# ffahleraz/rllib-warehouse

Hardware: AMD Instinct MI355X
Metric: agent-steps/sec (aggregate) at B=65536 envs × 8 agents, 1/2/4/8 MI355X (higher is better)
Workload: dtype u8/u32 packed integer state, f32 rewards

## Files before the change

### rllib-warehouse_amd/csrc/device_vocab.h

```cpp
constexpr int BT = 256;
using PkCell = uint16_t;
constexpr uint32_t PKW = sizeof(PkCell);
constexpr uint32_t ROWB = PKW * BT;

enum Policy { POL_EXTERNAL = 0, POL_GREEDY = 1, POL_RANDOM = 2 };
enum Purpose : uint32_t { PUR_RESET = 1, PUR_REGEN = 2, PUR_POLICY = 3, PUR_RANDOM = 4 };
constexpr int PH_ALL = 0, PH_PRE = 1, PH_REGEN = 2, PH_POLICY = 3;
#ifdef WH_ABLATION
constexpr bool kAblationBuild = true;
#else
constexpr bool kAblationBuild = false;
#endif

#ifndef WH_OBS_EB0
#define WH_OBS_EB0 4
#endif
constexpr int kObsEB[4] = {WH_OBS_EB0, 8, 16, 64};
#ifndef WH_OBS_CHUNK
#define WH_OBS_CHUNK 1024
#endif
constexpr int kObsChunk = WH_OBS_CHUNK;
#ifndef WH_FUSE_ROWS_MAX
#define WH_FUSE_ROWS_MAX 4096
#endif
// ... 148 lines not shown
}

__device__ __forceinline__ uint32_t action_of(uint32_t d) {
  const short2v v = as_s2(d);
  return (uint32_t)(3 * ((int)v.x + 1) + ((int)v.y + 1));
}

#define WH_RARE(x) __builtin_expect(!!(x), 0)

#ifdef WH_PHASE_MARKS
#define WH_PHASE_MARK(name) asm volatile("; PHASE " #name ::: "memory")
#else
#define WH_PHASE_MARK(name) ((void)0)
#endif

template <class C>
struct Regs {
  uint32_t hdr, epi;
  uint32_t ag[C::NAM];
  uint64_t am;
  uint32_t wskip;
};

template <class C>
struct Lds {
  alignas(16) uint32_t tbl[4 * C::TBL4];
  uint32_t occ[C::D][BT];
  PkCell pkp[C::P + 1][BT];
  alignas(16) uint32_t agl[C::NAM][BT];
  __device__ __forceinline__ uint32_t cell_row(uint32_t xy16) const {
    if constexpr (cell_skew(C::D)) {
      const uint32_t i = __builtin_amdgcn_udot4(xy16, 0x00840004u, 0u, false);
      return reinterpret_cast<const uint8_t*>(tbl)[i];
    } else {
      return reinterpret_cast<const uint8_t*>(tbl)[__builtin_amdgcn_perm(xy16, xy16, 0x0C0C0200u)];
    }
  }

  __device__ __forceinline__ uint2 rtag(uint32_t j) const {
    return reinterpret_cast<const uint2*>(&tbl[C::T.rp / 4])[j];
  }
  __device__ __forceinline__ uint32_t mv(uint32_t a) const { return tbl[C::T.mv / 4 + a]; }
  __device__ __forceinline__ uint32_t valid_cell(uint32_t v) const { return tbl[C::T.valid / 4 + v]; }
  __device__ __forceinline__ uint32_t target_byte(uint32_t j, int tid) const {
    return *reinterpret_cast<const uint8_t*>(&pkp[j][tid]);
  }
  __device__ __forceinline__ void clear_target(uint32_t j, int tid) {
    *reinterpret_cast<uint8_t*>(&pkp[j][tid]) = 0;
  }
  __device__ __forceinline__ uint32_t pkp_offset() const {
    return (uint32_t)(reinterpret_cast<const char*>(&pkp[0][0]) - reinterpret_cast<const char*>(this));
  }
  __device__ __forceinline__ const uint8_t* row_byte(uint32_t cv, int tid) const {
    return reinterpret_cast<const uint8_t*>(this) + (pkp_offset() - ROWB) + cv * ROWB + PKW * tid;
  }
  __device__ __forceinline__ uint8_t* row_byte(uint32_t cv, int tid) {
    return reinterpret_cast<uint8_t*>(this) + (pkp_offset() - ROWB) + cv * ROWB + PKW * tid;
  }
  __device__ __forceinline__ uint32_t dst_tb(uint32_t tb) const { return tbl[C::T.dst / 4 - 1 + tb]; }
};

template <class C>
struct Slots {
  uint32_t rs_ag[C::NAM][BT];
  uint16_t rs_req[C::R][BT];
  uint32_t rs_am[2][BT], rs_hdr[BT], rs_ep[BT];
};
struct NoSlots {};

template <class C>
constexpr int kTableChunks = (C::TBL4 + BT - 1) / BT;
template <class C>
__device__ __forceinline__ bool table_lane(int i) {
// ... 76 lines not shown
  for (int w = 0; w < C::PW; ++w) {
    const uint32_t lo = __builtin_amdgcn_perm(r.pm[w], r.pt[w], 0x05010400u);
    const uint32_t hi = __builtin_amdgcn_perm(r.pm[w], r.pt[w], 0x07030602u);
    L.pkp[4 * w][tid] = (uint16_t)lo;
    L.pkp[4 * w + 1][tid] = (uint16_t)(lo >> 16);
    L.pkp[4 * w + 2][tid] = (uint16_t)hi;
    L.pkp[4 * w + 3][tid] = (uint16_t)(hi >> 16);
  }
  s.am = active_mask<C>(r.pt);
  const uint32_t t0 = s.hdr & 0xFFFFu;
  const uint32_t thr = t0 < W ? W - t0 : 0u;
  uint32_t early = 0;
#pragma unroll
  for (int w = 0; w < C::PW; ++w)
    early |= nz_hi(r.pt[w]) & swar_lt(swar_sub(r.pm[w], (t0 & 0xFFu) * 0x01010101u), thr * 0x01010101u);
  s.wskip = __any(early != 0u) ? 0u : W;
}

template <class C>
__device__ __forceinline__ void store_env(const Regs<C>& s, const Lds<C>& L, uint32_t* __restrict__ st,
                                          int64_t B, int64_t e0, int na, int tid) {
  uint32_t* pl = st + e0;
  pl[tid] = s.hdr;
  pl += B;
  pl[tid] = s.epi;
#pragma unroll
  for (int i = 0; i < C::NAM; ++i)
    if (i < na) {
      pl += B;
      pl[tid] = s.ag[i];
    }
// ... 13 lines not shown
```

### rllib-warehouse_amd/csrc/policy.h

```cpp
template <class C>
__device__ __forceinline__ void policy_walk(const Regs<C>& s, const Lds<C>& L, uint32_t (&rp)[C::R],
                                            uint32_t (&tg)[C::R]) {
  const uint32_t mf = 0u - ((s.hdr >> 24) & 1u);
  uint32_t mlo = bop3<~TA & TB>(mf, (uint32_t)s.am, 0u);
  uint32_t mhi = bop3<~TA & TB>(mf, (uint32_t)(s.am >> 32), 0u);
#pragma unroll
  for (int r = 0; r < C::R; ++r) {
    uint32_t flo, fhi;
    asm("v_ffbl_b32 %0, %1" : "=v"(flo) : "v"(mlo));
    asm("v_ffbl_b32 %0, %1" : "=v"(fhi) : "v"(mhi));
    const uint32_t j = __builtin_elementwise_min(
        __builtin_elementwise_min(flo, __builtin_elementwise_add_sat(fhi, 32u)), (uint32_t)C::P);
    const uint2 v = L.rtag(j);
    rp[r] = v.x;
    tg[r] = v.y;
    uint64_t m = ((uint64_t)mhi << 32) | mlo;
    m &= m - 1ull;
    mlo = (uint32_t)m;
    mhi = (uint32_t)(m >> 32);
  }
}

template <class C, int POLICY, bool EFF = false, bool WALKED = false>
__device__ __forceinline__ void policy_steps(const Regs<C>& s, const Lds<C>& L, const Keys& k,
                                             uint32_t gid, float p, uint32_t (&d)[C::NAM],
                                             uint32_t (*walk_rp)[C::R] = nullptr,
                                             uint32_t (*walk_tg)[C::R] = nullptr) {
  const uint32_t t = s.hdr & 0xFFFFu;
  if (POLICY == POL_RANDOM) {
#pragma unroll
    for (int b = 0; b < (C::NAM + 3) / 4; ++b) {
      const uint4 blk = stream_block(k, gid, s.epi, t, PUR_RANDOM, (uint32_t)b);
#pragma unroll
      for (int c = 0; c < 4; ++c) {
        const int i = 4 * b + c;
        if (i < C::NAM) d[i] = L.mv(__umulhi(comp(blk, c), 9u));
      }
    }
// ... 12 lines not shown
    WH_PHASE_MARK(policy_agents);
#pragma unroll
    for (int i = 0; i < C::NAM; ++i) {
      const uint32_t a = s.ag[i];
      const uint32_t pos = a & XY16;
      uint32_t best = 0xFFFFFFFFu;
#pragma unroll
      for (int r = 0; r < C::R; ++r)
        best = min(best, __builtin_amdgcn_sad_hi_u8(pos, rp[r], tg[r]));
      const uint32_t near = (__builtin_amdgcn_ubfe(best, 5u, 5u) << 16) | (best & 31u);
      const uint32_t dst = __builtin_amdgcn_perm(a, a, 0x0C030C01u);
      const uint32_t idle = (uint32_t)__builtin_amdgcn_sbfe((int)a, 15, 1);
      const uint32_t goal = msel(idle, near, dst);
      d[i] = pk_min_i16(pk_max_i16(pk_sub_i16(goal, pos), 0xFFFFFFFFu), 0x00010001u);
    }
    if (WH_RARE(p > 0.0f)) {
#pragma unroll
      for (int b = 0; b < (C::NAM + 1) / 2; ++b) {
        const uint4 blk = stream_block(k, gid, s.epi, t, PUR_POLICY, (uint32_t)b);
#pragma unroll
        for (int h = 0; h < 2; ++h) {
          const int i = 2 * b + h;
          if (i < C::NAM) {
            const float u = (float)(comp(blk, 2 * h) >> 8) * (1.0f / 16777216.0f);
            uint32_t rnd = L.mv(__umulhi(comp(blk, 2 * h + 1), 9u));
            if (EFF) {
              const uint32_t pos = s.ag[i] & XY16;
              rnd = pk_sub_i16(step16<C::D>(pos, rnd), pos);
            }
            d[i] = (u < p) ? rnd : d[i];
          }
// ... 6 lines not shown
```

### rllib-warehouse_amd/csrc/step_env.h

```cpp
struct LazyGrid {
  bool rebuild;
  uint32_t cm;
};

#ifdef WH_COUNT_REV
__device__ unsigned long long g_wh_revcount[2];
#endif

struct OrderIn {
  const int32_t* __restrict__ order;
  int ol;
  uint16_t* keys;
};
template <class C>
struct OKeys {
  uint16_t k[4 * C::NAM][BT];
};

template <class C, bool ORDERED, bool INJ = true, bool CLAMP = true, bool LAZY = false>
__device__ __forceinline__ bool step_env(Regs<C>& s, Lds<C>& L, const uint32_t (&dstep)[C::NAM],
                                         const OrderIn& oi,
                                         const int32_t* __restrict__ actions_g,
                                         const int32_t* __restrict__ regen, const Keys& k,
                                         uint32_t gid, int64_t e, int na, int phase, uint32_t T,
                                         uint32_t W, float (&rew)[C::NAM], int32_t* n_inactive,
                                         int tid, int ablate, LazyGrid* lg = nullptr,
                                         const uint4* pre_rblk = nullptr) {
  const uint32_t n = (s.hdr >> 16) & 0xFFu;
  uint32_t t = s.hdr & 0xFFFFu;
  uint32_t rewm[C::NAM];
  const uint4 rblk0 = pre_rblk ? *pre_rblk : make_uint4(0u, 0u, 0u, 0u);

  if (phase != PH_REGEN) {
    t = (t + 1u) & 0xFFFFu;
#pragma unroll
    for (int i = 0; i < C::NAM; ++i) rewm[i] = 0u;

    WH_PHASE_MARK(expire);
    const uint64_t em = (ablate & 4) ? 0ull : __ballot(t >= s.wskip);
    if (WH_RARE(em != 0) && __popcll(em) == 1 && __ballot(true) == ~0ull) {
      const int l = __builtin_ctzll(em), lane = tid & 63, col = (tid & ~63) + l;
      const uint32_t t8 = (uint32_t)__builtin_amdgcn_readlane(t, l) & 0xFFu;
// ... 54 lines not shown
      clr[i] = msel(m, cpv, (uint32_t)(C::P + 1));
      rewm[i] = m;
    };
    if (!(ablate & 2)) {
      if (ORDERED) {
#pragma unroll
        for (int y = 0; y < C::D; ++y) L.occ[y][tid] = 0u;
      }
      if (!LAZY) {
#pragma unroll
        for (int i = 0; i < C::NAM; ++i) {
          const uint32_t p = s.ag[i] & XY16;
          const uint32_t mlive = sgn((uint32_t)i - n);
          atomicOr(&L.occ[p >> 16][tid], bop3<TA & TB>(mlive, 1u << (p & 31u), 0u));
        }
      } else if (WH_RARE(__any(lg->rebuild))) {
        const uint32_t livebits = (2u << (n - 1u)) - 1u;
        uint32_t q[C::NAM];
#pragma unroll
        for (int i = 0; i < C::NAM; ++i) {
          const uint32_t a = s.ag[i];
          const uint32_t mlive = (uint32_t)__builtin_amdgcn_sbfe((int)livebits, (uint32_t)i, 1u);
          uint32_t bit;
          asm volatile("v_lshlrev_b32 %0, %1, 1" : "=v"(bit) : "v"(a));
          atomicOr(&L.occ[__builtin_amdgcn_ubfe(a, 16u, 8u)][tid], bop3<TA & TB>(mlive, bit, 0u));
          q[i] = msel(mlive, a, 0x80u + (uint32_t)i);
        }
        uint32_t m[C::NAM];
#pragma unroll
        for (int i = 0; i < C::NAM; ++i) m[i] = 0xFFFFFFFFu;
#pragma unroll
        for (int i = 1; i < C::NAM; ++i)
#pragma unroll
          for (int j = 0; j < i; ++j) {
            const uint32_t x = bop3<(TA ^ TB) & TC>(q[i], q[j], XY16);
            m[i] = min(m[i], x);
            m[j] = min(m[j], x);
          }
        uint32_t cm = 0;
#pragma unroll
        for (int i = 0; i < C::NAM; ++i) cm |= (m[i] == 0u ? 1u : 0u) << i;
        lg->cm = cm;
        lg->rebuild = false;
      }
      if (ORDERED) {
#pragma unroll
        for (int i = 0; i < C::NAM; ++i) L.agl[i][tid] = s.ag[i];
        auto entry = [&](int sidx, int32_t raw, bool unrolled) {
          int who = raw < 0 ? -1 : (raw & 0xFF);
          const uint32_t sact = raw < 0 ? 0u : ((uint32_t)raw >> 8) & 0xFFu;
          const bool live = who >= 0 && who < (int)n && who < C::NAM;
          who = live ? who : 0;
          const uint32_t a = L.agl[who][tid];
          const uint32_t mv = live ? (sact ? sact - 1u : (uint32_t)actions_g[e * na + who]) : 4u;
          const uint32_t p = a & XY16;
          const uint32_t c = step16<C::D>(p, L.mv(mv > 8u ? 4u : mv));
          const bool occupied = (L.occ[c >> 16][tid] >> (c & 31u)) & 1u;
// ... 49 lines not shown
            const uint32_t p = pp[sidx], c = cc[sidx], a = s.ag[sidx];
            uint32_t occ31 = (uint32_t)__builtin_amdgcn_sbfe((int)raw, c, 1);
            if (sidx >= 1) {
              const int j = sidx - 1;
              const uint32_t set31 = (c ^ cc[j]) - 1u;
              const uint32_t clr31 = (c ^ pp[j]) - 1u;
              occ31 = bop3<(TA & TB) | (TC & ~(TA & TB))>(mokh[j], set31, bop3<TC & ~(TA & TB)>(mokh[j], clr31, occ31));
            }
            if (sidx + 1 < C::NAM) raw = *occ_at(cc[sidx + 1 < C::NAM ? sidx + 1 : 0]);
            const uint32_t dd = CLAMP ? pk_sub_i16(c, p) : dstep[sidx];
            const uint32_t kpr = __builtin_amdgcn_perm(as_u(as_s2(p) + as_s2(c)), dd, 0x06040200u);
            uint32_t f = 0xFFFFu;
#pragma unroll
            for (int j = 0; j < sidx; ++j) f = min(f, (kpr ^ sk[j]) - 1u);
            f -= 0xFFFEu;
            const uint32_t live31 = (uint32_t)sidx - n;
            const uint32_t mok = sgn(bop3<TA & ~TB & ~TC>(live31, occ31, f - 1u));
            atomicAnd(occ_at(p), bop3<~(TA & TB)>(mok, 1u << (p & 31u), 0u));
            atomicOr(occ_at(c), bop3<TA & TB>(mok, 1u << (c & 31u), 0u));
            const uint32_t dxy = c ^ p;
            if constexpr (REV) {
              uint32_t z;
              asm("v_ffbl_b32 %0, %1" : "=v"(z) : "v"(dd));
              sk[sidx] = bop3<~TA | (TB ^ TC)>(mok, kpr, z >> 31);
            } else {
              sk[sidx] = bop3<~TA | (TB ^ TC)>(mok, kpr, 1u);
            }
            const uint32_t moved = bop3<TA ^ (TB & TC)>(a, mok, dxy);
            s.ag[sidx] = moved;
            mokh[sidx] = mok;
            constexpr int PD = kPickDist;
            cp[sidx] = L.cell_row(moved);
            if (sidx >= PD) tb[sidx - PD] = *L.row_byte(cp[sidx >= PD ? sidx - PD : 0], tid);
            if (sidx >= 2 * PD) dst[sidx - 2 * PD] = L.dst_tb(tb[sidx >= 2 * PD ? sidx - 2 * PD : 0]);
            if (!(ablate & 8) && sidx >= 3 * PD) {
              const int j = sidx >= 3 * PD ? sidx - 3 * PD : 0;
              pick(j, cp[j], tb[j], dst[j]);
            }
          }
        };
        auto shared_moved = [&]() {
          uint32_t acc = 0;
#pragma unroll
          for (int i = 0; i < C::NAM; ++i)
            acc |= (s.ag[i] ^ pp[i]) & (XY16 & (uint32_t)__builtin_amdgcn_sbfe((int)lg->cm, (uint32_t)i, 1u));
          lg->rebuild = lg->rebuild || acc != 0u;
        };
#ifdef WH_NO_PICK_MERGE
        constexpr bool CM_IN_REV = false;
#else
        constexpr bool CM_IN_REV = LAZY && C::NAM <= kRevSplitMaxNam;
#endif
        if (!LAZY || C::NAM > kRevSplitMaxNam || WH_RARE(__any(lg->cm != 0u))) {
#ifdef WH_COUNT_REV
          if (LAZY && __lane_id() == 0) atomicAdd(&g_wh_revcount[0], 1ull);
#endif
          move_loop(std::true_type{});
          if constexpr (CM_IN_REV) shared_moved();
        } else {
#ifdef WH_COUNT_REV
          if (__lane_id() == 0) atomicAdd(&g_wh_revcount[1], 1ull);
#endif
          move_loop(std::false_type{});
        }
        constexpr int PD = kPickDist;
#pragma unroll
        for (int i = (C::NAM > PD ? C::NAM - PD : 0); i < C::NAM; ++i) tb[i] = *L.row_byte(cp[i], tid);
#pragma unroll
        for (int i = (C::NAM > 2 * PD ? C::NAM - 2 * PD : 0); i < C::NAM; ++i) dst[i] = L.dst_tb(tb[i]);
        if (!(ablate & 8)) {
#pragma unroll
          for (int i = (C::NAM > 3 * PD ? C::NAM - 3 * PD : 0); i < C::NAM; ++i) pick(i, cp[i], tb[i], dst[i]);
        }
        looked = true;
        if constexpr (LAZY && !CM_IN_REV) {
          if (WH_RARE(__any(lg->cm != 0u))) shared_moved();
        }
      }
    }

    WH_PHASE_MARK(pickup);
    if (!(ablate & 8)) {
      if (!looked) {
#pragma unroll
        for (int i = 0; i < C::NAM; ++i) cp[i] = L.cell_row(s.ag[i]);
#pragma unroll
        for (int i = 0; i < C::NAM; ++i) tb[i] = *L.row_byte(cp[i], tid);
#pragma unroll
        for (int i = 0; i < C::NAM; ++i) dst[i] = L.dst_tb(tb[i]);
#pragma unroll
        for (int i = 0; i < C::NAM; ++i) pick(i, cp[i], tb[i], dst[i]);
      }
#pragma unroll
      for (int i = 0; i < C::NAM; ++i) *L.row_byte(clr[i], tid) = 0;
      const uint64_t pr = ((uint64_t)prhi << 32) | prlo;
      s.am &= ~((pr >> 1) | (pr << 63));
    }
  }

  WH_PHASE_MARK(regen);
  if (!(ablate & 16)) {
    const uint64_t inactive = ~s.am & low_mask<C::P>();
// ... 71 lines not shown
#pragma unroll
    for (int i = 0; i < C::NAM; ++i) delm[i] = 0u;
    if (!(ablate & 32)) {
#pragma unroll
      for (int i = 0; i < C::NAM; ++i) {
        const uint32_t a = s.ag[i];
        const uint32_t m = sgn(__builtin_amdgcn_sad_u8(a, __builtin_amdgcn_perm(a, a, 0x03030101u), 0xFFFFFFFFu));
        s.ag[i] = bop3<(TA & TB) | TC>(m, IDLE, a);
        delm[i] = m;
      }
    }
#pragma unroll
    for (int i = 0; i < C::NAM; ++i) rew[i] = __uint_as_float(bop3<(TA | TB) & TC>(rewm[i], delm[i], 0x3F800000u));
    WH_PHASE_MARK(tail);
    done = t >= T;
    s.hdr = t | (n << 16);
  }
  return done;
}

template <int R, int A0 = 1, int G0 = 1 + R, int P0 = 1 + 3 * R, int Q0 = 1 + 5 * R>
__host__ __device__ constexpr uint32_t obs_src(int i, int f, bool fresh) {
  if (f == 0) return 0;
  if (f < R) {
    const int j = f - 1;
    return A0 + (j < i ? j : j + 1);
  }
  if (f < 3 * R - 2) {
    const int k = f - R, j = k >> 1, drop = fresh ? i : 1;
    return G0 + 2 * (j < drop ? j : j + 1) + (k & 1);
  }
// ... 100 lines not shown
```

### rllib-warehouse_amd/csrc/step_loops.h

```cpp

#ifdef WH_ABLATION
#define WH_ABLATE_WORD(a) ((a).ablate)
#else
#define WH_ABLATE_WORD(a) 0
#endif

template <class C>
__device__ __forceinline__ uint32_t move_of(const Lds<C>& L, uint32_t action) {
  return L.mv(action > 8u ? 4u : action);
}

template <class C>
__device__ __forceinline__ void ablation_moves(const Lds<C>& L, int stp, uint32_t (&d)[C::NAM]) {
#pragma unroll
  for (int i = 0; i < C::NAM; ++i) d[i] = L.mv((uint32_t)((i + stp) % 9));
}

template <class C, int POLICY, bool ORDERED, int PHASE>
__device__ __forceinline__ void run_steps(const StepParams& a, Regs<C>& s, Lds<C>& L, const Keys& k,
                                          uint32_t gid, int64_t e, int tid, uint16_t* okeys = nullptr) {
  const int phase = PHASE >= 0 ? PHASE : a.phase;
  const OrderIn oi{a.order, a.ol, okeys};
  const int ablate = WH_ABLATE_WORD(a);
  float ret = 0.0f;
// ... 56 lines not shown
  } else {
#pragma unroll
    for (int q = 0; q < C::NAM / 2; ++q) reinterpret_cast<float2*>(row)[q] = make_float2(rew[2 * q], rew[2 * q + 1]);
  }
}


template <class C, int POLICY, bool SLOTS = true>
struct FastRun {
  float* rrow;
  uint8_t* drow;
  int64_t rstride;
  LazyGrid lg;
  uint32_t act[POLICY == POL_EXTERNAL ? C::NAM : 1];
  __device__ __forceinline__ FastRun(const StepParams& a, int64_t e)
      : rrow(a.rewards + e * C::NAM), drow(a.dones + e), rstride(a.B * C::NAM), lg{true, 0u} {}
  __device__ __forceinline__ void load_actions(const StepParams& a, int64_t e) {
    if constexpr (POLICY == POL_EXTERNAL) {
      if constexpr (C::NAM % 4 == 0) {
        const uint4* src = reinterpret_cast<const uint4*>(a.actions + e * C::NAM);
#pragma unroll
        for (int q = 0; q < C::NAM / 4; ++q) {
          const uint4 v = src[q];
          act[4 * q] = v.x; act[4 * q + 1] = v.y; act[4 * q + 2] = v.z; act[4 * q + 3] = v.w;
        }
      } else {
        const uint2* src = reinterpret_cast<const uint2*>(a.actions + e * C::NAM);
#pragma unroll
        for (int q = 0; q < C::NAM / 2; ++q) {
          const uint2 v = src[q];
          act[2 * q] = v.x; act[2 * q + 1] = v.y;
// ... 14 lines not shown
    } else {
      policy_steps<C, POLICY, POLICY == POL_GREEDY && !kAblationBuild>(s, L, k, gid, a.p, d);
    }
    float rew[C::NAM];
    const bool done = step_env<C, false, false, POLICY != POL_GREEDY || kAblationBuild, true>(s, L, d, OrderIn{nullptr, 0, nullptr}, nullptr, nullptr, k, gid, e, C::NAM, PH_ALL,
                                                (uint32_t)a.T, (uint32_t)a.W, rew, nullptr, tid, ablate, &lg);
    if (!(ablate & 64)) {
      store_row<C>(rrow, rew);
      *drow = done ? 1 : 0;
    }
    rrow += rstride;
    drow += a.B;
    if (!(ablate & 128) && WH_RARE(__any(done))) {
      const uint64_t dm = __ballot(done);
      const bool full = __ballot(true) == ~0ull;
      if (SLOTS && a.steps >= kSlotMinSteps && __popcll(dm) <= kSlotResetMax && full) {
        if constexpr (SLOTS) {
          if (__any(done && RS->rs_ep[tid] != s.epi + 1u))
            reset_philox<C, C::NAM, true>(s, L, k, gid, C::NAM, a.variable_n, (uint32_t)a.W, tid, RS);
          for (uint64_t m = dm; m; m &= m - 1ull) reset_from_slot<C, C::NAM>(s, L, *RS, (uint32_t)a.W, tid, __builtin_ctzll(m));
          lg.rebuild = lg.rebuild || done;
        }
      } else if (__popcll(dm) == 1 && full) {
        reset_lane<C, C::NAM>(s, L, k, gid, a.variable_n, (uint32_t)a.W, tid, __builtin_ctzll(dm));
        lg.rebuild = lg.rebuild || done;
      } else if (dm == ~0ull) {
        reset_philox<C, C::NAM, false, true>(s, L, k, gid, C::NAM, a.variable_n, (uint32_t)a.W, tid);
        lg.rebuild = true;
      } else if (done) {
        reset_philox<C, C::NAM>(s, L, k, gid, C::NAM, a.variable_n, (uint32_t)a.W, tid);
#pragma unroll
        for (int y = 0; y < C::D; ++y) L.occ[y][tid] = 0u;
        lg.rebuild = true;
      }
    }
    WH_CHECK_ENV(s, L, e, tid);
  }
};

template <class C, int POLICY, bool SLOTS = true>
__device__ __forceinline__ void run_steps_fast(const StepParams& a, Regs<C>& s, Lds<C>& L, Slots<C>* RS,
                                               const Keys& k, uint32_t gid, int64_t e, int tid) {
  const int ablate = WH_ABLATE_WORD(a);
  float* rrow = a.rewards + (e - tid) * C::NAM;
  uint8_t* drow = a.dones + (e - tid);
  const int64_t rstride = a.B * C::NAM;
  LazyGrid lg{true, 0u};
  constexpr bool ROT = kWalkRotate && POLICY == POL_GREEDY && !kAblationBuild;
  [[maybe_unused]] uint32_t wrp[C::R], wtg[C::R];
  if constexpr (ROT) policy_walk<C>(s, L, wrp, wtg);
  for (int stp = 0; stp < a.steps; ++stp) {
    uint32_t d[C::NAM];
    if constexpr (POLICY == POL_EXTERNAL) {
#pragma unroll
      for (int i = 0; i < C::NAM; ++i) d[i] = move_of<C>(L, (uint32_t)a.actions[e * C::NAM + i]);
    } else if (ablate & 1) {
      ablation_moves<C>(L, stp, d);
    } else if constexpr (ROT) {
      policy_steps<C, POLICY, true, true>(s, L, k, gid, a.p, d, &wrp, &wtg);
    } else {
      policy_steps<C, POLICY, POLICY == POL_GREEDY && !kAblationBuild>(s, L, k, gid, a.p, d);
    }
    uint4 rb = stream_block(k, gid, s.epi, (s.hdr + 1u) & 0xFFFFu, PUR_REGEN, 0u);
    asm volatile("" : "+v"(rb.x), "+v"(rb.y), "+v"(rb.z), "+v"(rb.w));
    float rew[C::NAM];
    const bool done = step_env<C, false, false, POLICY != POL_GREEDY || kAblationBuild, true>(s, L, d, OrderIn{nullptr, 0, nullptr}, nullptr, nullptr, k, gid, e, C::NAM, PH_ALL,
                                                (uint32_t)a.T, (uint32_t)a.W, rew, nullptr, tid, ablate, &lg,
                                                &rb);
    if constexpr (ROT) policy_walk<C>(s, L, wrp, wtg);
    if (!(ablate & 64)) {
      store_row<C>(rrow + tid * C::NAM, rew);
      drow[tid] = done ? 1 : 0;
    }
    rrow += rstride;
    drow += a.B;
    if (!(ablate & 128) && WH_RARE(__any(done))) {
      const uint64_t dm = __ballot(done);
      const bool full = __ballot(true) == ~0ull;
      if (SLOTS && a.steps >= kSlotMinSteps && __popcll(dm) <= kSlotResetMax && full) {
        if constexpr (SLOTS) {
          if (__any(done && RS->rs_ep[tid] != s.epi + 1u))
            reset_philox<C, C::NAM, true>(s, L, k, gid, C::NAM, a.variable_n, (uint32_t)a.W, tid, RS);
          for (uint64_t m = dm; m; m &= m - 1ull) reset_from_slot<C, C::NAM>(s, L, *RS, (uint32_t)a.W, tid, __builtin_ctzll(m));
          lg.rebuild = lg.rebuild || done;
        }
      } else if (__popcll(dm) == 1 && full) {
        reset_lane<C, C::NAM>(s, L, k, gid, a.variable_n, (uint32_t)a.W, tid, __builtin_ctzll(dm));
        lg.rebuild = lg.rebuild || done;
      } else if (dm == ~0ull) {
        reset_philox<C, C::NAM, false, true>(s, L, k, gid, C::NAM, a.variable_n, (uint32_t)a.W, tid);
        lg.rebuild = true;
      } else if (done) {
        reset_philox<C, C::NAM>(s, L, k, gid, C::NAM, a.variable_n, (uint32_t)a.W, tid);
#pragma unroll
        for (int y = 0; y < C::D; ++y) L.occ[y][tid] = 0u;
        lg.rebuild = true;
      }
      if constexpr (ROT) policy_walk<C>(s, L, wrp, wtg);
    }
    WH_CHECK_ENV(s, L, e, tid);
  }
}


#ifdef WH_TIMING
constexpr int kTimeSlots = 6, kTimeWaves = 4096;
__device__ unsigned long long g_wh_times[kTimeWaves * kTimeSlots];
#define WH_T(i)                                                                                   \
  do {                                                                                            \
    const unsigned long long now_ = __builtin_amdgcn_s_memrealtime();                             \
    const int w_ = (int)blockIdx.x * (BT / 64) + (int)(threadIdx.x >> 6);                        \
    if ((threadIdx.x & 63) == 0 && w_ < kTimeWaves) g_wh_times[w_ * kTimeSlots + (i)] = now_;     \
  } while (0)
#else
#define WH_T(i) ((void)0)
#endif

template <class C, int POLICY, bool ORDERED, bool FAST>
__global__ __launch_bounds__(BT) void k_step(StepParams a) {
  __shared__ Lds<C> L;
  __shared__ std::conditional_t<FAST, Slots<C>, NoSlots> RS;
  __shared__ std::conditional_t<ORDERED, OKeys<C>, NoSlots> OK;
  const int tid = threadIdx.x;
  if (FAST) WH_T(0);
  const int64_t e = (int64_t)blockIdx.x * BT + tid;
  const bool live = e < a.B && (FAST || !a.mask || a.mask[e]);
  const int na = FAST ? C::NAM : a.na;
  const int64_t e0 = (int64_t)blockIdx.x * BT;
  const uint4 tv0 = issue_table_chunk<C>(a.tables, 0), tv1 = issue_table_chunk<C>(a.tables, 1);
  __builtin_amdgcn_sched_barrier(0);
  RawEnv<C> raw;
  load_env_issue<C>(raw, a.state, a.B, e0, live ? tid : 0, na);
  commit_table_chunk<C>(L.tbl, 0, tv0);
  commit_table_chunk<C>(L.tbl, 1, tv1);
// ... 13 lines not shown
  __builtin_amdgcn_s_waitcnt(0x0F70);
  if constexpr (FAST) RS.rs_ep[tid] = s.epi;
  if (FAST) WH_T(2);

  if (!FAST && a.phase == PH_POLICY) {
    uint32_t d[C::NAM];
    policy_steps<C, POLICY>(s, L, k, gid, a.p, d);
    const uint32_t n = (s.hdr >> 16) & 0xFFu;
#pragma unroll
    for (int i = 0; i < C::NAM; ++i)
      if (i < a.na) a.actions_out[e * a.na + i] = (i < (int)n) ? (int32_t)action_of(d[i]) : 4;
    return;
  }

  if constexpr (FAST)
    run_steps_fast<C, POLICY>(a, s, L, &RS, k, gid, e, tid);
  else if (!ORDERED && a.phase == PH_ALL)
    run_steps<C, POLICY, ORDERED, PH_ALL>(a, s, L, k, gid, e, tid);
  else if constexpr (ORDERED)
    run_steps<C, POLICY, ORDERED, -1>(a, s, L, k, gid, e, tid, &OK.k[0][0]);
  else
    run_steps<C, POLICY, ORDERED, -1>(a, s, L, k, gid, e, tid);
  if (FAST) WH_T(3);
  store_env<C>(s, L, a.state_out ? a.state_out : a.state, a.B, e0, na, tid);
#ifdef WH_TIMING
  if (FAST) {
    __builtin_amdgcn_s_waitcnt(0);
    WH_T(4);
  }
#endif
}
// ... 33 lines not shown
```

### rllib-warehouse_amd/csrc/warehouse_amd.hip

```cpp
#include <hip/hip_ext.h>
#include <hip/hip_runtime.h>

#include <mutex>
#include <type_traits>
#include <unordered_set>
#include <new>
#include <stdint.h>
#include <stdlib.h>
#include <string.h>
#include <vector>

#include "abi_args.h"
#include "geometry.h"
#include "philox.h"
#include "sac_formula.h"
#include "warehouse_amd.h"

namespace {

#include "device_vocab.h"
#include "reset.h"
#include "policy.h"
#include "step_env.h"
#include "step_params.h"
// ... 82 lines not shown
  if (he == hipSuccess) he = hipMemset(d, 0, padded);
  if (he == hipSuccess) he = hipMemcpy(d, w.data(), w.size() * 4, hipMemcpyHostToDevice);
  if (cur != dev) (void)hipSetDevice(cur);
  if (he != hipSuccess) return hip_err(he);
  TableEntry t{dev, g.D, g.NR, (int)w.size(), {0}, d};
  memcpy(t.racks, g.racks, sizeof(int) * g.NR);
  g_tabs.push_back(t);
  *out = d;
  return WH_OK;
}

struct Kernels {
  int D, R, NR, NAM;
  void (*step[3])(StepParams);
  void (*step_fast[3])(StepParams);
  void (*step_ordered)(StepParams);
  void (*step_wide[3])(StepParams);
  void (*sampler[3])(StepParams, float*);
  void (*sampler_multi[3])(StepParams, float*);
  void (*vsampler[2])(StepParams, float*);
  void (*reset)(ResetParams);
  void (*observe[4])(const uint32_t*, int64_t, int, const uint32_t*, float*, int, uint4*);
  void (*observe_chunk)(const uint32_t*, int64_t, int, const uint32_t*, float*, int, uint4*);
  void (*replay_put)(PutParams);
  void (*replay_gather[4])(GatherParams);
  int tblw, nv;
};

template <class C>
constexpr bool kSamplerBuilt = C::R < 16 || WH_FUSE_ROWS_MAX > 4096;

template <int D, int R, int NR, int NAM>
Kernels make_kernels() {
  using C = Cfg<D, R, NR, NAM>;
  Kernels k;
  k.D = D; k.R = R; k.NR = NR; k.NAM = NAM;
  k.step[0] = k_step<C, POL_EXTERNAL, false, false>;
  k.step[1] = k_step<C, POL_GREEDY, false, false>;
  k.step[2] = k_step<C, POL_RANDOM, false, false>;
  k.step_fast[0] = nullptr;
  k.sampler[0] = k.sampler[1] = k.sampler[2] = nullptr;
  k.sampler_multi[0] = k.sampler_multi[1] = k.sampler_multi[2] = nullptr;
  constexpr bool sampler_fits = sizeof(Lds<C>) + sizeof(Slots<C>) + sizeof(SampLds<C, 2>) <= 160 * 1024;
  if constexpr (NAM % 2 == 0) {
    k.step_fast[0] = k_step<C, POL_EXTERNAL, false, true>;
    k.step_fast[1] = k_step<C, POL_GREEDY, false, true>;
    k.step_fast[2] = k_step<C, POL_RANDOM, false, true>;
    if constexpr (kSamplerBuilt<C>) {
      k.sampler[0] = k_sampler<C, POL_EXTERNAL, false, true>;
      k.sampler[1] = k_sampler<C, POL_GREEDY, false, true>;
      k.sampler[2] = k_sampler<C, POL_RANDOM, false, true>;
    }
    if constexpr (sampler_fits && kSamplerBuilt<C>) {
      k.sampler_multi[1] = k_sampler<C, POL_GREEDY, false, true, true>;
      k.sampler_multi[2] = k_sampler<C, POL_RANDOM, false, true, true>;
    }
  } else {
    k.step_fast[1] = k.step_fast[2] = nullptr;
  }
  static_assert(sizeof(Lds<C>) + sizeof(OKeys<C>) <= 160 * 1024, "k_step<..., ORDERED> exceeds the LDS of a workgroup");
  k.step_ordered = k_step<C, POL_EXTERNAL, true, false>;
  k.step_wide[0] = k_step_wide<C, POL_EXTERNAL>;
// ... 235 lines not shown
  return a;
}

static int resolve_step(const StepCall& c, void* stream, wh_launch* out) {
  const uint32_t* tab;
  const int rc = locate(c.g, c.B, stream, &out->k, &tab);
  if (rc) return rc;
  const Kernels* k = out->k;
  const int policy = c.policy;
  const StepParams a = step_params(c, tab);
  void (*kern)(StepParams) = (a.order != nullptr && policy == POL_EXTERNAL) ? k->step_ordered : k->step[policy];
  const uintptr_t ralign = (k->NAM % 4 == 0) ? 15u : 7u;
  if (k->step_fast[policy] && a.phase == PH_ALL && a.rewards && a.dones && !a.returns &&
      !a.stats.episode_return && !a.mask && !a.order && !a.regen && !a.n_inactive && a.autoreset &&
      c.g.NA == k->NAM && ((uintptr_t)a.rewards & ralign) == 0)
    kern = k->step_fast[policy];
  const bool wide = c.lanes == WH_WIDE_LANES;
  out->kern = wide ? k->step_wide[policy] : kern;
  out->grid = wide ? grid_wide(c.B) : grid_for(c.B);
  out->stream = (hipStream_t)stream;
  out->a = a;
  out->g = c.g;
  return WH_OK;
}

static int enqueue(const wh_launch& l) {
  if (l.a.B == 0) return WH_OK;
  hipLaunchKernelGGL(l.kern, l.grid, dim3(BT), 0, l.stream, l.a);
  return hip_err(hipGetLastError());
}

static int launch_step(const StepCall& c, void* stream) {
  wh_launch l;
  const int rc = resolve_step(c, stream, &l);
  return rc ? rc : enqueue(l);
}

static int obs_group_sel(const Geometry& g, bool rows, bool frags) {
// ... 45 lines not shown
  if (rc || c.B == 0) return rc;
  if (c.lanes == 1 && c.obs) {
    void (*fk)(StepParams, float*) =
        (l.kern == l.k->step_fast[0] && l.k->sampler[0]) ? l.k->sampler[0] : l.k->vsampler[c.order ? 1 : 0];
    if (rows_fusable(l, fk, c.obs)) return enqueue_fused(l, fk, c.obs);
  }
  rc = enqueue(l);
  if (rc || (!c.obs && !c.xfrag)) return rc;
  return observe_launch(l.g, l.k, l.a.tables, c.B, c.state, c.obs, c.xfrag, stream);
}

static int sampler_step(const StepCall& c, void* stream) {
  wh_launch l;
  int rc = resolve_step(c, stream, &l);
  if (rc || c.B == 0) return rc;
  if (l.kern == l.k->step_fast[c.policy] && rows_fusable(l, l.k->sampler[c.policy], c.obs))
    return enqueue_fused(l, l.k->sampler[c.policy], c.obs);
  rc = enqueue(l);
  if (rc || !c.obs) return rc;
  return observe_launch(l.g, l.k, l.a.tables, c.B, c.state, c.obs, nullptr, stream);
}

extern "C" {

int wh_step(const wh_config* cfg, int64_t B, uint32_t* state, const int32_t* actions,
            const int32_t* order, int32_t order_len, float* rewards, uint8_t* dones, const int32_t* regen,
            int32_t* n_inactive, int32_t phase, uint64_t seed, int64_t env_offset, void* stream) {
  StepCall c;
  const int rc = wh_abi::step_call(&c, cfg, B, state, actions, order, order_len, rewards, dones, regen, n_inactive,
                                   phase, seed, env_offset, 1);
  return rc ? rc : launch_step(c, stream);
// ... 105 lines not shown
                                           variable_n, seed, env_offset);
  return rc ? rc : sampler_step(c, stream);
}

int wh_sampler_rollout(const wh_config* cfg, int64_t B, uint32_t* state, int32_t steps, int32_t policy, float p,
                       float* rewards, uint8_t* dones, float* obs, const wh_episode_stats* stats, int32_t variable_n,
                       uint64_t seed, int64_t env_offset, void* stream) {
  StepCall c;
  int rc = wh_abi::sampler_rollout_call(&c, cfg, B, state, steps, policy, p, rewards, dones, obs, stats, variable_n,
                                        seed, env_offset);
  if (rc) return rc;
  wh_launch l;
  rc = resolve_step(c, stream, &l);
  if (rc || B == 0 || steps == 0) return rc;
  void (*fk)(StepParams, float*) = steps == 1 ? l.k->sampler[policy] : l.k->sampler_multi[policy];
  if (l.kern == l.k->step_fast[policy] && rows_fusable(l, fk, obs)) return enqueue_fused(l, fk, obs);
  c.steps = 1;
  for (int32_t t = 0; t < steps && rc == WH_OK; ++t) {
    rc = sampler_step(c, stream);
    if (c.rewards) c.rewards += B * c.g.NA;
    if (c.dones) c.dones += B;
    c.obs += B * c.g.NA * c.g.L;
  }
  return rc;
}

int wh_sampler_step_to(const wh_config* cfg, int64_t B, const uint32_t* state_in, uint32_t* state_out,
                       int32_t policy, float p, float* rewards, uint8_t* dones, const wh_episode_stats* stats,
                       int32_t variable_n, uint64_t seed, int64_t env_offset, void* stream) {
  StepCall c;
  const int rc = wh_abi::sampler_step_call(&c, cfg, B, state_in, state_out, true, policy, p, rewards, dones, nullptr,
// ... 158 lines not shown
```

Baseline: 261.7 billion.

## Add eps-free greedy fast kernel and hoist per-env constants, wave-uniform lazy flags

Adds a compile-time EPS=false specialisation of the fast greedy step kernel and selects it on the host when p is zero, removing the epsilon-exploration branch and its RNG code. It also caches per-env live masks and header bits in an EnvConst struct that is refreshed only after resets. The lazy-grid rebuild and shared flags are made wave-uniform once instead of being re-evaluated with __any on every step. LDS byte loads go through an opaque asm barrier, and the walk skips mask filtering after a step. These cut VALU work and register pressure in the hot loop, at the cost of an extra kernel instantiation and more subtle invariants around when the flags are recomputed.

Result: faster. 272.5 billion (median of 6 runs) (+4.1%).

```diff
diff --git a/rllib-warehouse_amd/csrc/device_vocab.h b/rllib-warehouse_amd/csrc/device_vocab.h
--- a/rllib-warehouse_amd/csrc/device_vocab.h
+++ b/rllib-warehouse_amd/csrc/device_vocab.h
@@ -186,6 +186,14 @@
 #define WH_PHASE_MARK(name) ((void)0)
 #endif
 
+__device__ __forceinline__ uint32_t lds_byte(const uint8_t* p) {
+  uint32_t v = *p;
+#ifndef WH_NO_BYTE_OPAQUE
+  asm("" : "+v"(v));
+#endif
+  return v;
+}
+
 template <class C>
 struct Regs {
   uint32_t hdr, epi;
@@ -203,9 +211,9 @@
   __device__ __forceinline__ uint32_t cell_row(uint32_t xy16) const {
     if constexpr (cell_skew(C::D)) {
       const uint32_t i = __builtin_amdgcn_udot4(xy16, 0x00840004u, 0u, false);
-      return reinterpret_cast<const uint8_t*>(tbl)[i];
+      return lds_byte(reinterpret_cast<const uint8_t*>(tbl) + i);
     } else {
-      return reinterpret_cast<const uint8_t*>(tbl)[__builtin_amdgcn_perm(xy16, xy16, 0x0C0C0200u)];
+      return lds_byte(reinterpret_cast<const uint8_t*>(tbl) + __builtin_amdgcn_perm(xy16, xy16, 0x0C0C0200u));
     }
   }
 
@@ -229,6 +237,7 @@
   __device__ __forceinline__ uint8_t* row_byte(uint32_t cv, int tid) {
     return reinterpret_cast<uint8_t*>(this) + (pkp_offset() - ROWB) + cv * ROWB + PKW * tid;
   }
+  __device__ __forceinline__ uint32_t row_target(uint32_t cv, int tid) const { return lds_byte(row_byte(cv, tid)); }
   __device__ __forceinline__ uint32_t dst_tb(uint32_t tb) const { return tbl[C::T.dst / 4 - 1 + tb]; }
 };
 
@@ -335,7 +344,11 @@
 #pragma unroll
   for (int w = 0; w < C::PW; ++w)
     early |= nz_hi(r.pt[w]) & swar_lt(swar_sub(r.pm[w], (t0 & 0xFFu) * 0x01010101u), thr * 0x01010101u);
+#ifdef WH_WSKIP_SCALAR
+  s.wskip = (uint32_t)__builtin_amdgcn_readfirstlane((int)(__any(early != 0u) ? 0u : W));
+#else
   s.wskip = __any(early != 0u) ? 0u : W;
+#endif
 }
 
 template <class C>
diff --git a/rllib-warehouse_amd/csrc/policy.h b/rllib-warehouse_amd/csrc/policy.h
--- a/rllib-warehouse_amd/csrc/policy.h
+++ b/rllib-warehouse_amd/csrc/policy.h
@@ -1,9 +1,9 @@
-template <class C>
+template <class C, bool STEPPED = false>
 __device__ __forceinline__ void policy_walk(const Regs<C>& s, const Lds<C>& L, uint32_t (&rp)[C::R],
                                             uint32_t (&tg)[C::R]) {
   const uint32_t mf = 0u - ((s.hdr >> 24) & 1u);
-  uint32_t mlo = bop3<~TA & TB>(mf, (uint32_t)s.am, 0u);
-  uint32_t mhi = bop3<~TA & TB>(mf, (uint32_t)(s.am >> 32), 0u);
+  uint32_t mlo = STEPPED ? (uint32_t)s.am : bop3<~TA & TB>(mf, (uint32_t)s.am, 0u);
+  uint32_t mhi = STEPPED ? (uint32_t)(s.am >> 32) : bop3<~TA & TB>(mf, (uint32_t)(s.am >> 32), 0u);
 #pragma unroll
   for (int r = 0; r < C::R; ++r) {
     uint32_t flo, fhi;
@@ -21,7 +21,7 @@
   }
 }
 
-template <class C, int POLICY, bool EFF = false, bool WALKED = false>
+template <class C, int POLICY, bool EFF = false, bool WALKED = false, bool EPS = true>
 __device__ __forceinline__ void policy_steps(const Regs<C>& s, const Lds<C>& L, const Keys& k,
                                              uint32_t gid, float p, uint32_t (&d)[C::NAM],
                                              uint32_t (*walk_rp)[C::R] = nullptr,
@@ -64,7 +64,7 @@
       const uint32_t goal = msel(idle, near, dst);
       d[i] = pk_min_i16(pk_max_i16(pk_sub_i16(goal, pos), 0xFFFFFFFFu), 0x00010001u);
     }
-    if (WH_RARE(p > 0.0f)) {
+    if (EPS && WH_RARE(p > 0.0f)) {
 #pragma unroll
       for (int b = 0; b < (C::NAM + 1) / 2; ++b) {
         const uint4 blk = stream_block(k, gid, s.epi, t, PUR_POLICY, (uint32_t)b);
diff --git a/rllib-warehouse_amd/csrc/step_env.h b/rllib-warehouse_amd/csrc/step_env.h
--- a/rllib-warehouse_amd/csrc/step_env.h
+++ b/rllib-warehouse_amd/csrc/step_env.h
@@ -1,6 +1,19 @@
 struct LazyGrid {
   bool rebuild;
   uint32_t cm;
+  bool shared;
+};
+
+template <class C>
+struct EnvConst {
+  uint32_t live31[C::NAM];
+  uint32_t n16;
+  __device__ __forceinline__ void set(uint32_t hdr) {
+    const uint32_t n = (hdr >> 16) & 0xFFu;
+#pragma unroll
+    for (int i = 0; i < C::NAM; ++i) live31[i] = (uint32_t)i - n;
+    n16 = n << 16;
+  }
 };
 
 #ifdef WH_COUNT_REV
@@ -25,7 +38,8 @@
                                          uint32_t gid, int64_t e, int na, int phase, uint32_t T,
                                          uint32_t W, float (&rew)[C::NAM], int32_t* n_inactive,
                                          int tid, int ablate, LazyGrid* lg = nullptr,
-                                         const uint4* pre_rblk = nullptr) {
+                                         const uint4* pre_rblk = nullptr,
+                                         const EnvConst<C>* ec = nullptr) {
   const uint32_t n = (s.hdr >> 16) & 0xFFu;
   uint32_t t = s.hdr & 0xFFFFu;
   uint32_t rewm[C::NAM];
@@ -110,7 +124,7 @@
           const uint32_t mlive = sgn((uint32_t)i - n);
           atomicOr(&L.occ[p >> 16][tid], bop3<TA & TB>(mlive, 1u << (p & 31u), 0u));
         }
-      } else if (WH_RARE(__any(lg->rebuild))) {
+      } else if (WH_RARE(lg->rebuild)) {
         const uint32_t livebits = (2u << (n - 1u)) - 1u;
         uint32_t q[C::NAM];
 #pragma unroll
@@ -137,6 +151,7 @@
 #pragma unroll
         for (int i = 0; i < C::NAM; ++i) cm |= (m[i] == 0u ? 1u : 0u) << i;
         lg->cm = cm;
+        lg->shared = __any(cm != 0u);
         lg->rebuild = false;
       }
       if (ORDERED) {
@@ -216,7 +231,7 @@
 #pragma unroll
             for (int j = 0; j < sidx; ++j) f = min(f, (kpr ^ sk[j]) - 1u);
             f -= 0xFFFEu;
-            const uint32_t live31 = (uint32_t)sidx - n;
+            const uint32_t live31 = ec ? ec->live31[sidx] : (uint32_t)sidx - n;
             const uint32_t mok = sgn(bop3<TA & ~TB & ~TC>(live31, occ31, f - 1u));
             atomicAnd(occ_at(p), bop3<~(TA & TB)>(mok, 1u << (p & 31u), 0u));
             atomicOr(occ_at(c), bop3<TA & TB>(mok, 1u << (c & 31u), 0u));
@@ -233,7 +248,7 @@
             mokh[sidx] = mok;
             constexpr int PD = kPickDist;
             cp[sidx] = L.cell_row(moved);
-            if (sidx >= PD) tb[sidx - PD] = *L.row_byte(cp[sidx >= PD ? sidx - PD : 0], tid);
+            if (sidx >= PD) tb[sidx - PD] = L.row_target(cp[sidx >= PD ? sidx - PD : 0], tid);
             if (sidx >= 2 * PD) dst[sidx - 2 * PD] = L.dst_tb(tb[sidx >= 2 * PD ? sidx - 2 * PD : 0]);
             if (!(ablate & 8) && sidx >= 3 * PD) {
               const int j = sidx >= 3 * PD ? sidx - 3 * PD : 0;
@@ -246,14 +261,14 @@
 #pragma unroll
           for (int i = 0; i < C::NAM; ++i)
             acc |= (s.ag[i] ^ pp[i]) & (XY16 & (uint32_t)__builtin_amdgcn_sbfe((int)lg->cm, (uint32_t)i, 1u));
-          lg->rebuild = lg->rebuild || acc != 0u;
+          lg->rebuild = lg->rebuild || __any(acc != 0u);
         };
 #ifdef WH_NO_PICK_MERGE
         constexpr bool CM_IN_REV = false;
 #else
         constexpr bool CM_IN_REV = LAZY && C::NAM <= kRevSplitMaxNam;
 #endif
-        if (!LAZY || C::NAM > kRevSplitMaxNam || WH_RARE(__any(lg->cm != 0u))) {
+        if (!LAZY || C::NAM > kRevSplitMaxNam || WH_RARE(lg->shared)) {
 #ifdef WH_COUNT_REV
           if (LAZY && __lane_id() == 0) atomicAdd(&g_wh_revcount[0], 1ull);
 #endif
@@ -267,7 +282,7 @@
         }
         constexpr int PD = kPickDist;
 #pragma unroll
-        for (int i = (C::NAM > PD ? C::NAM - PD : 0); i < C::NAM; ++i) tb[i] = *L.row_byte(cp[i], tid);
+        for (int i = (C::NAM > PD ? C::NAM - PD : 0); i < C::NAM; ++i) tb[i] = L.row_target(cp[i], tid);
 #pragma unroll
         for (int i = (C::NAM > 2 * PD ? C::NAM - 2 * PD : 0); i < C::NAM; ++i) dst[i] = L.dst_tb(tb[i]);
         if (!(ablate & 8)) {
@@ -276,7 +291,7 @@
         }
         looked = true;
         if constexpr (LAZY && !CM_IN_REV) {
-          if (WH_RARE(__any(lg->cm != 0u))) shared_moved();
+          if (WH_RARE(lg->shared)) shared_moved();
         }
       }
     }
@@ -287,7 +302,7 @@
 #pragma unroll
         for (int i = 0; i < C::NAM; ++i) cp[i] = L.cell_row(s.ag[i]);
 #pragma unroll
-        for (int i = 0; i < C::NAM; ++i) tb[i] = *L.row_byte(cp[i], tid);
+        for (int i = 0; i < C::NAM; ++i) tb[i] = L.row_target(cp[i], tid);
 #pragma unroll
         for (int i = 0; i < C::NAM; ++i) dst[i] = L.dst_tb(tb[i]);
 #pragma unroll
@@ -389,7 +404,7 @@
     for (int i = 0; i < C::NAM; ++i) rew[i] = __uint_as_float(bop3<(TA | TB) & TC>(rewm[i], delm[i], 0x3F800000u));
     WH_PHASE_MARK(tail);
     done = t >= T;
-    s.hdr = t | (n << 16);
+    s.hdr = t | (ec ? ec->n16 : n << 16);
   }
   return done;
 }
diff --git a/rllib-warehouse_amd/csrc/step_loops.h b/rllib-warehouse_amd/csrc/step_loops.h
--- a/rllib-warehouse_amd/csrc/step_loops.h
+++ b/rllib-warehouse_amd/csrc/step_loops.h
@@ -94,7 +94,7 @@
   LazyGrid lg;
   uint32_t act[POLICY == POL_EXTERNAL ? C::NAM : 1];
   __device__ __forceinline__ FastRun(const StepParams& a, int64_t e)
-      : rrow(a.rewards + e * C::NAM), drow(a.dones + e), rstride(a.B * C::NAM), lg{true, 0u} {}
+      : rrow(a.rewards + e * C::NAM), drow(a.dones + e), rstride(a.B * C::NAM), lg{true, 0u, false} {}
   __device__ __forceinline__ void load_actions(const StepParams& a, int64_t e) {
     if constexpr (POLICY == POL_EXTERNAL) {
       if constexpr (C::NAM % 4 == 0) {
@@ -139,38 +139,37 @@
     if (!(ablate & 128) && WH_RARE(__any(done))) {
       const uint64_t dm = __ballot(done);
       const bool full = __ballot(true) == ~0ull;
+      lg.rebuild = true;
       if (SLOTS && a.steps >= kSlotMinSteps && __popcll(dm) <= kSlotResetMax && full) {
         if constexpr (SLOTS) {
           if (__any(done && RS->rs_ep[tid] != s.epi + 1u))
             reset_philox<C, C::NAM, true>(s, L, k, gid, C::NAM, a.variable_n, (uint32_t)a.W, tid, RS);
           for (uint64_t m = dm; m; m &= m - 1ull) reset_from_slot<C, C::NAM>(s, L, *RS, (uint32_t)a.W, tid, __builtin_ctzll(m));
-          lg.rebuild = lg.rebuild || done;
         }
       } else if (__popcll(dm) == 1 && full) {
         reset_lane<C, C::NAM>(s, L, k, gid, a.variable_n, (uint32_t)a.W, tid, __builtin_ctzll(dm));
-        lg.rebuild = lg.rebuild || done;
       } else if (dm == ~0ull) {
         reset_philox<C, C::NAM, false, true>(s, L, k, gid, C::NAM, a.variable_n, (uint32_t)a.W, tid);
-        lg.rebuild = true;
       } else if (done) {
         reset_philox<C, C::NAM>(s, L, k, gid, C::NAM, a.variable_n, (uint32_t)a.W, tid);
 #pragma unroll
         for (int y = 0; y < C::D; ++y) L.occ[y][tid] = 0u;
-        lg.rebuild = true;
       }
     }
     WH_CHECK_ENV(s, L, e, tid);
   }
 };
 
-template <class C, int POLICY, bool SLOTS = true>
+template <class C, int POLICY, bool SLOTS = true, bool EPS = true>
 __device__ __forceinline__ void run_steps_fast(const StepParams& a, Regs<C>& s, Lds<C>& L, Slots<C>* RS,
                                                const Keys& k, uint32_t gid, int64_t e, int tid) {
   const int ablate = WH_ABLATE_WORD(a);
   float* rrow = a.rewards + (e - tid) * C::NAM;
   uint8_t* drow = a.dones + (e - tid);
   const int64_t rstride = a.B * C::NAM;
-  LazyGrid lg{true, 0u};
+  LazyGrid lg{true, 0u, false};
+  EnvConst<C> ec;
+  ec.set(s.hdr);
   constexpr bool ROT = kWalkRotate && POLICY == POL_GREEDY && !kAblationBuild;
   [[maybe_unused]] uint32_t wrp[C::R], wtg[C::R];
   if constexpr (ROT) policy_walk<C>(s, L, wrp, wtg);
@@ -182,17 +181,21 @@
     } else if (ablate & 1) {
       ablation_moves<C>(L, stp, d);
     } else if constexpr (ROT) {
-      policy_steps<C, POLICY, true, true>(s, L, k, gid, a.p, d, &wrp, &wtg);
+      policy_steps<C, POLICY, true, true, EPS>(s, L, k, gid, a.p, d, &wrp, &wtg);
     } else {
-      policy_steps<C, POLICY, POLICY == POL_GREEDY && !kAblationBuild>(s, L, k, gid, a.p, d);
+      policy_steps<C, POLICY, POLICY == POL_GREEDY && !kAblationBuild, false, EPS>(s, L, k, gid, a.p, d);
     }
     uint4 rb = stream_block(k, gid, s.epi, (s.hdr + 1u) & 0xFFFFu, PUR_REGEN, 0u);
     asm volatile("" : "+v"(rb.x), "+v"(rb.y), "+v"(rb.z), "+v"(rb.w));
     float rew[C::NAM];
     const bool done = step_env<C, false, false, POLICY != POL_GREEDY || kAblationBuild, true>(s, L, d, OrderIn{nullptr, 0, nullptr}, nullptr, nullptr, k, gid, e, C::NAM, PH_ALL,
                                                 (uint32_t)a.T, (uint32_t)a.W, rew, nullptr, tid, ablate, &lg,
+#ifndef WH_NO_ENV_CONST
+                                                &rb, &ec);
+#else
                                                 &rb);
-    if constexpr (ROT) policy_walk<C>(s, L, wrp, wtg);
+#endif
+    if constexpr (ROT) policy_walk<C, true>(s, L, wrp, wtg);
     if (!(ablate & 64)) {
       store_row<C>(rrow + tid * C::NAM, rew);
       drow[tid] = done ? 1 : 0;
@@ -202,26 +205,24 @@
     if (!(ablate & 128) && WH_RARE(__any(done))) {
       const uint64_t dm = __ballot(done);
       const bool full = __ballot(true) == ~0ull;
+      lg.rebuild = true;
       if (SLOTS && a.steps >= kSlotMinSteps && __popcll(dm) <= kSlotResetMax && full) {
         if constexpr (SLOTS) {
           if (__any(done && RS->rs_ep[tid] != s.epi + 1u))
             reset_philox<C, C::NAM, true>(s, L, k, gid, C::NAM, a.variable_n, (uint32_t)a.W, tid, RS);
           for (uint64_t m = dm; m; m &= m - 1ull) reset_from_slot<C, C::NAM>(s, L, *RS, (uint32_t)a.W, tid, __builtin_ctzll(m));
-          lg.rebuild = lg.rebuild || done;
         }
       } else if (__popcll(dm) == 1 && full) {
         reset_lane<C, C::NAM>(s, L, k, gid, a.variable_n, (uint32_t)a.W, tid, __builtin_ctzll(dm));
-        lg.rebuild = lg.rebuild || done;
       } else if (dm == ~0ull) {
         reset_philox<C, C::NAM, false, true>(s, L, k, gid, C::NAM, a.variable_n, (uint32_t)a.W, tid);
-        lg.rebuild = true;
       } else if (done) {
         reset_philox<C, C::NAM>(s, L, k, gid, C::NAM, a.variable_n, (uint32_t)a.W, tid);
 #pragma unroll
         for (int y = 0; y < C::D; ++y) L.occ[y][tid] = 0u;
-        lg.rebuild = true;
       }
       if constexpr (ROT) policy_walk<C>(s, L, wrp, wtg);
+      ec.set(s.hdr);
     }
     WH_CHECK_ENV(s, L, e, tid);
   }
@@ -241,8 +242,9 @@
 #define WH_T(i) ((void)0)
 #endif
 
-template <class C, int POLICY, bool ORDERED, bool FAST>
+template <class C, int POLICY, bool ORDERED, bool FAST, bool EPS = true>
 __global__ __launch_bounds__(BT) void k_step(StepParams a) {
+  static_assert(EPS || (FAST && POLICY == POL_GREEDY), "the eps = 0 form exists for the fused greedy rollout only");
   __shared__ Lds<C> L;
   __shared__ std::conditional_t<FAST, Slots<C>, NoSlots> RS;
   __shared__ std::conditional_t<ORDERED, OKeys<C>, NoSlots> OK;
@@ -286,7 +288,7 @@
   }
 
   if constexpr (FAST)
-    run_steps_fast<C, POLICY>(a, s, L, &RS, k, gid, e, tid);
+    run_steps_fast<C, POLICY, true, EPS>(a, s, L, &RS, k, gid, e, tid);
   else if (!ORDERED && a.phase == PH_ALL)
     run_steps<C, POLICY, ORDERED, PH_ALL>(a, s, L, k, gid, e, tid);
   else if constexpr (ORDERED)
diff --git a/rllib-warehouse_amd/csrc/warehouse_amd.hip b/rllib-warehouse_amd/csrc/warehouse_amd.hip
--- a/rllib-warehouse_amd/csrc/warehouse_amd.hip
+++ b/rllib-warehouse_amd/csrc/warehouse_amd.hip
@@ -120,6 +120,7 @@
   int D, R, NR, NAM;
   void (*step[3])(StepParams);
   void (*step_fast[3])(StepParams);
+  void (*step_fast_eps0)(StepParams);
   void (*step_ordered)(StepParams);
   void (*step_wide[3])(StepParams);
   void (*sampler[3])(StepParams, float*);
@@ -145,6 +146,7 @@
   k.step[1] = k_step<C, POL_GREEDY, false, false>;
   k.step[2] = k_step<C, POL_RANDOM, false, false>;
   k.step_fast[0] = nullptr;
+  k.step_fast_eps0 = nullptr;
   k.sampler[0] = k.sampler[1] = k.sampler[2] = nullptr;
   k.sampler_multi[0] = k.sampler_multi[1] = k.sampler_multi[2] = nullptr;
   constexpr bool sampler_fits = sizeof(Lds<C>) + sizeof(Slots<C>) + sizeof(SampLds<C, 2>) <= 160 * 1024;
@@ -152,6 +154,7 @@
     k.step_fast[0] = k_step<C, POL_EXTERNAL, false, true>;
     k.step_fast[1] = k_step<C, POL_GREEDY, false, true>;
     k.step_fast[2] = k_step<C, POL_RANDOM, false, true>;
+    k.step_fast_eps0 = k_step<C, POL_GREEDY, false, true, false>;
     if constexpr (kSamplerBuilt<C>) {
       k.sampler[0] = k_sampler<C, POL_EXTERNAL, false, true>;
       k.sampler[1] = k_sampler<C, POL_GREEDY, false, true>;
@@ -417,7 +420,11 @@
   if (k->step_fast[policy] && a.phase == PH_ALL && a.rewards && a.dones && !a.returns &&
       !a.stats.episode_return && !a.mask && !a.order && !a.regen && !a.n_inactive && a.autoreset &&
       c.g.NA == k->NAM && ((uintptr_t)a.rewards & ralign) == 0)
+#ifndef WH_NO_EPS0
+    kern = (policy == POL_GREEDY && !(a.p > 0.0f)) ? k->step_fast_eps0 : k->step_fast[policy];
+#else
     kern = k->step_fast[policy];
+#endif
   const bool wide = c.lanes == WH_WIDE_LANES;
   out->kern = wide ? k->step_wide[policy] : kern;
   out->grid = wide ? grid_wide(c.B) : grid_for(c.B);
@@ -425,6 +432,10 @@
   out->a = a;
   out->g = c.g;
   return WH_OK;
+}
+
+static bool fast_step(const wh_launch& l, int policy) {
+  return l.kern == l.k->step_fast[policy] || (policy == POL_GREEDY && l.k->step_fast_eps0 && l.kern == l.k->step_fast_eps0);
 }
 
 static int enqueue(const wh_launch& l) {
@@ -500,7 +511,7 @@
   wh_launch l;
   int rc = resolve_step(c, stream, &l);
   if (rc || c.B == 0) return rc;
-  if (l.kern == l.k->step_fast[c.policy] && rows_fusable(l, l.k->sampler[c.policy], c.obs))
+  if (fast_step(l, c.policy) && rows_fusable(l, l.k->sampler[c.policy], c.obs))
     return enqueue_fused(l, l.k->sampler[c.policy], c.obs);
   rc = enqueue(l);
   if (rc || !c.obs) return rc;
@@ -636,7 +647,7 @@
   rc = resolve_step(c, stream, &l);
   if (rc || B == 0 || steps == 0) return rc;
   void (*fk)(StepParams, float*) = steps == 1 ? l.k->sampler[policy] : l.k->sampler_multi[policy];
-  if (l.kern == l.k->step_fast[policy] && rows_fusable(l, fk, obs)) return enqueue_fused(l, fk, obs);
+  if (fast_step(l, policy) && rows_fusable(l, fk, obs)) return enqueue_fused(l, fk, obs);
   c.steps = 1;
   for (int32_t t = 0; t < steps && rc == WH_OK; ++t) {
     rc = sampler_step(c, stream);
```
